# cambridge-mlg/RECOMBINER

Measured on AMD Instinct MI355X. Metric: INRs trained/sec (whole node) + PSNR@bpp vs reference, CIFAR-10, higher is better.
Workload: dtype bf16; 1 GPU; CIFAR-10 32x32, 4096 INRs/GPU, 3x32 SIREN (in 32 = 16 Fourier + 16 upsampled pe), S=1, training_mappings=True, Adam lr 2e-4; inrs_per_gpu=4096, parallelism=datapoint-sharded x1, tuned_library_gemms=True

## Files before the change

### recombiner_amd/csrc/atrans.hip

```cpp
#include "rcb_common.h"
#include "prepare_bodies.h"

#include <algorithm>
#include <type_traits>
#include <vector>

using namespace rcb;

namespace {

typedef __bf16 bf16x8 __attribute__((ext_vector_type(8)));
typedef float f32x16 __attribute__((ext_vector_type(16)));
typedef float f32x4 __attribute__((ext_vector_type(4)));

#ifndef ATRANS_DIAG
#define ATRANS_DIAG 0
#endif
#ifndef ATRANS_STAMPS
#define ATRANS_STAMPS 0
#endif
#ifndef ATRANS_SPREAD_PIN
#define ATRANS_SPREAD_PIN 1
#endif
constexpr int BM = 256, BK = 32, NT = 512, MAXL = RCB_ATRANS_MAX_LAYERS, MAXSEG = 7;
constexpr int XT_BYTES = BM * BK * 4;

__device__ __forceinline__ constexpr int rho(int r, int h) { return (r & 3) + 8 * (r >> 2) + 4 * h; }
__device__ __forceinline__ int xswz(int row, int c) { return row * 128 + ((c ^ ((row >> 1) & 7)) << 4); }
__device__ __forceinline__ int bswz(int row, int c) { return row * 64 + ((c ^ ((row >> 2) & 3)) << 4); }

typedef __attribute__((address_space(3))) void* lds_ptr_t;
__device__ __forceinline__ void dma16(const void* g, char* l) {
  __builtin_amdgcn_global_load_lds(g, (lds_ptr_t)l, 16, 0, 0);
}
__device__ __forceinline__ f32x16 mma(bf16x8 a, bf16x8 b, f32x16 c) {
#if ATRANS_DIAG == 4
  asm volatile("" ::"v"(a), "v"(b));
  return c;
#else
  return __builtin_amdgcn_mfma_f32_32x32x16_bf16(a, b, c, 0, 0, 0);
#endif
}
template <int N>
__device__ __forceinline__ void wait_vm() { asm volatile("s_waitcnt vmcnt(%0)" ::"n"(N) : "memory"); }
#if ATRANS_STAMPS
__device__ unsigned long long g_stamps[8][40][6];
#define STAMP(it, pt)                                                                 \
  do {                                                                               \
    if (blockIdx.x == 0 && (it) < 40) {                                              \
      const unsigned long long t_ = __builtin_amdgcn_s_memtime();                    \
      if (lane == 0) g_stamps[wave][it][pt] = t_;                                    \
    }                                                                                \
  } while (0)
#else
#define STAMP(it, pt)
#endif

struct AtArgs {
  const float* x;
  const __bf16* xh;
  const __bf16* xl;
  long long ld_x16;
  float* out;
  long long ld_x, ld_out, rows;
  int n_layers;
  int L[MAXL], Lp[MAXL], off[MAXL];
  const __bf16* bh[MAXL];
  const __bf16* bl[MAXL];
  const int4* segs;
  const int* seg_begin;
  int n_wg;
  int nt_out;
  float* ws;
  long long ld_ws;
};

template <int NCB, int TERMS>
struct Geo {
  static constexpr int NBW = (2 * NCB + 7) / 8;
  static constexpr int NDMA = 4 + NBW * (TERMS == 3 ? 2 : 1);
  static constexpr int BH_OFF = XT_BYTES;
  static constexpr int BT_BYTES = NCB * 32 * BK * 2;
  static constexpr int BL_OFF = BH_OFF + BT_BYTES;
  static constexpr int STAGE = BH_OFF + (TERMS == 3 ? 2 : 1) * BT_BYTES;
  static constexpr int NSTAGE = TERMS == 3 ? 2 : 3;
};
constexpr int LDS_MAX_BYTES = 3 * (XT_BYTES + MAXSEG * 32 * BK * 2);

template <int NCB, int TERMS, bool RAGGED, bool PLANES>
__device__ __forceinline__ void run_segment(const AtArgs& a, const int4 sg, const int4 sk, char* __restrict__ lds) {
  typedef Geo<NCB, TERMS> G;
  const int t = threadIdx.x, lane = t & 63;
  const int wave = __builtin_amdgcn_readfirstlane(t >> 6);
  const int l = sg.x, row0 = sg.y, cb0 = sg.z, ncb = sg.w;
  const int K = a.L[l], Lp = a.Lp[l];
  const int kc0 = sk.x, nk = sk.y - sk.x;
  const __bf16* __restrict__ bh = a.bh[l];
  const __bf16* __restrict__ bl = a.bl[l];
  const float* __restrict__ xl0 = PLANES ? nullptr : a.x + a.off[l];

  f32x16 acc[NCB];
#pragma unroll
  for (int i = 0; i < NCB; ++i)
#pragma unroll
    for (int q = 0; q < 16; ++q) acc[i][q] = 0.f;

  const float* xsrc[4];
  const __bf16* psrc[4];
  int xk[4];
#pragma unroll
  for (int i = 0; i < 4; ++i) {
    if (PLANES) {
      const int row = 32 * wave + 16 * (i & 1) + (lane >> 2);
      const int c = (lane & 3) ^ ((row >> 2) & 3);
      const long long gr = min((long long)row0 + row, a.rows - 1);
      psrc[i] = ((i >> 1) ? a.xl : a.xh) + gr * a.ld_x16 + a.off[l];
      xk[i] = 8 * c;
      xsrc[i] = nullptr;
    } else {
      const int row = 32 * wave + 8 * i + (lane >> 3);
      const int c = (lane & 7) ^ ((row >> 1) & 7);
      const long long gr = min((long long)row0 + row, a.rows - 1);
      xsrc[i] = xl0 + gr * a.ld_x;
      xk[i] = 4 * c;
      psrc[i] = nullptr;
    }
  }
  const __bf16* bsrc[G::NBW];
  const __bf16* bsrc2[G::NBW];
  int bdst[G::NBW];
#pragma unroll
  for (int j = 0; j < G::NBW; ++j) {
    const int d = min(wave + 8 * j, 2 * NCB - 1);
    const int row = 16 * d + (lane >> 2);
    const int c = (lane & 3) ^ ((row >> 2) & 3);
    const int grow = min(cb0 * 32 + row, Lp - 1);
    bsrc[j] = bh + (long long)grow * Lp + 8 * c;
    bsrc2[j] = bl + (long long)grow * Lp + 8 * c;
    bdst[j] = __builtin_amdgcn_readfirstlane(d * 1024);
  }
  auto issue_one = [&](int kc_, int i) {
    char* __restrict__ st = lds + (kc_ % G::NSTAGE) * G::STAGE;
    const int kc = ATRANS_DIAG == 2 ? 0 : kc0 + kc_;
    if (i < 4) {
      if (PLANES) {
        const int k = RAGGED ? 0 : min(kc * BK + xk[i], K - 8);
        dma16(psrc[i] + k, st + (i >> 1) * (XT_BYTES / 2) + (32 * wave + 16 * (i & 1)) * 64);
      } else {
        const int k = RAGGED ? 0 : min(kc * BK + xk[i], K - 4);
        dma16(xsrc[i] + k, st + (32 * wave + 8 * i) * 128);
      }
    } else if (TERMS == 3) {
      const int j = (i - 4) >> 1;
      if ((i - 4) & 1) dma16(bsrc2[j] + kc * BK, st + G::BL_OFF + bdst[j]);
      else dma16(bsrc[j] + kc * BK, st + G::BH_OFF + bdst[j]);
    } else {
      dma16(bsrc[i - 4] + kc * BK, st + G::BH_OFF + bdst[i - 4]);
    }
  };
  auto issue = [&](int kc) {
#pragma unroll
    for (int i = 0; i < G::NDMA; ++i) issue_one(kc, i);
  };

  const int frow = lane & 31, fh = lane >> 5;
  const int xrow = 32 * wave + frow;
  bf16x8 xh[2], xlo[2];
  f32x4 raw[4];
  auto x_read = [&](const char* __restrict__ st) {
    if (PLANES) {
#pragma unroll
      for (int q = 0; q < 4; ++q)
        if (TERMS >= 2 || q < 2)
          raw[q] = *reinterpret_cast<const f32x4*>(st + (q >> 1) * (XT_BYTES / 2) + bswz(xrow, 2 * (q & 1) + fh));
    } else {
#pragma unroll
      for (int q = 0; q < 4; ++q) raw[q] = *reinterpret_cast<const f32x4*>(st + xswz(xrow, 4 * (q >> 1) + 2 * fh + (q & 1)));
    }
  };
  auto x_convert = [&](int q) {
    if (PLANES) {
      if (q < 2) xh[q] = __builtin_bit_cast(bf16x8, raw[q]);
      else if (TERMS >= 2) xlo[q - 2] = __builtin_bit_cast(bf16x8, raw[q]);
      return;
    }
#pragma unroll
    for (int i = 0; i < 4; ++i) {
      const float v = raw[q][i];
      const __bf16 hb = (__bf16)v;
      xh[q >> 1][4 * (q & 1) + i] = hb;
      if (TERMS >= 2) xlo[q >> 1][4 * (q & 1) + i] = (__bf16)(v - (float)hb);
    }
  };
  constexpr int NBT = G::NDMA - 4;
  constexpr int CBR = (NCB - 1) / 2;
  auto compute = [&](const char* __restrict__ cur, const char* __restrict__ nxt, int kn, auto issue_c, auto pref_c) {
    constexpr bool ISSUE = decltype(issue_c)::value, PREF = decltype(pref_c)::value;
    bf16x8 b0 = *reinterpret_cast<const bf16x8*>(cur + G::BH_OFF + bswz(frow, fh));
    bf16x8 b1 = *reinterpret_cast<const bf16x8*>(cur + G::BH_OFF + bswz(frow, 2 + fh));
#pragma unroll
    for (int cb = 0; cb < NCB; ++cb) {
      const bf16x8 c0 = b0, c1 = b1;
      if (cb + 1 < NCB) {
        b0 = *reinterpret_cast<const bf16x8*>(cur + G::BH_OFF + bswz((cb + 1) * 32 + frow, fh));
        b1 = *reinterpret_cast<const bf16x8*>(cur + G::BH_OFF + bswz((cb + 1) * 32 + frow, 2 + fh));
      }
      acc[cb] = mma(xh[0], c0, acc[cb]);
      if (TERMS >= 2) acc[cb] = mma(xlo[0], c0, acc[cb]);
      acc[cb] = mma(xh[1], c1, acc[cb]);
      if (TERMS >= 2) acc[cb] = mma(xlo[1], c1, acc[cb]);
      if (TERMS == 3) {
        const int bo0 = bswz(cb * 32 + frow, fh), bo1 = bswz(cb * 32 + frow, 2 + fh);
        const bf16x8 d0 = *reinterpret_cast<const bf16x8*>(cur + G::BL_OFF + bo0);
        const bf16x8 d1 = *reinterpret_cast<const bf16x8*>(cur + G::BL_OFF + bo1);
        acc[cb] = mma(xh[0], d0, acc[cb]);
        acc[cb] = mma(xh[1], d1, acc[cb]);
      }
      if (ISSUE && ATRANS_DIAG != 6) {
#pragma unroll
        for (int i = cb * G::NDMA / NCB; i < (cb + 1) * G::NDMA / NCB; ++i) issue_one(kn, i);
      }
      if (PREF) {
        if (cb == CBR) {
          STAMP(kn - 2, 3);
          wait_vm<NBT + (ISSUE ? (CBR + 1) * G::NDMA / NCB : 0)>();
          x_read(nxt);
        }
      }
#if ATRANS_SPREAD_PIN
      __builtin_amdgcn_sched_barrier(0);
#endif
    }
    if (PREF) {
      STAMP(kn - 2, 4);
#pragma unroll
      for (int q = 0; q < 4; ++q) x_convert(q);
    }
  };
  auto yes = std::integral_constant<bool, true>{};
  auto no = std::integral_constant<bool, false>{};

  if (RAGGED) {
    for (int kr = 0; kr < nk; ++kr) {
      const int kc = kc0 + kr;
      __syncthreads();
#pragma unroll
      for (int j = 0; j < G::NBW; ++j) {
        dma16(bsrc[j] + kc * BK, lds + G::BH_OFF + bdst[j]);
        if (TERMS == 3) dma16(bsrc2[j] + kc * BK, lds + G::BL_OFF + bdst[j]);
      }
#pragma unroll
      for (int i = 0; i < 4; ++i) {
        const int k0 = kc * BK + xk[i];
        if (PLANES) {
          const int row = 32 * wave + 16 * (i & 1) + (lane >> 2), pc = lane & 3;
          const bool rok = (long long)row0 + row < a.rows;
          bf16x8 v;
#pragma unroll
          for (int e = 0; e < 8; ++e) v[e] = (rok && k0 + e < K) ? psrc[i][k0 + e] : (__bf16)0.f;
          *reinterpret_cast<bf16x8*>(lds + (i >> 1) * (XT_BYTES / 2) + row * 64 + pc * 16) = v;
        } else {
          const int row = 32 * wave + 8 * i + (lane >> 3), pc = lane & 7;
          const bool rok = (long long)row0 + row < a.rows;
          f32x4 v;
#pragma unroll
          for (int e = 0; e < 4; ++e) v[e] = (rok && k0 + e < K) ? xsrc[i][k0 + e] : 0.f;
          *reinterpret_cast<f32x4*>(lds + row * 128 + pc * 16) = v;
        }
      }
      wait_vm<0>();
      __syncthreads();
      x_read(lds);
#pragma unroll
      for (int q = 0; q < 4; ++q) x_convert(q);
      compute(lds, lds, -1, no, no);
    }
    __syncthreads();
  } else if (G::NSTAGE == 2) {
    issue(0);
    for (int kc = 0; kc < nk; ++kc) {
      wait_vm<0>();
      __builtin_amdgcn_s_barrier();
      __builtin_amdgcn_sched_barrier(0);
      const char* cur = lds + (kc & 1) * G::STAGE;
      x_read(cur);
#pragma unroll
      for (int q = 0; q < 4; ++q) x_convert(q);
      if (kc + 1 < nk) compute(cur, cur, kc + 1, yes, no);
      else compute(cur, cur, -1, no, no);
    }
    __builtin_amdgcn_s_barrier();
  } else {
    issue(0);
    if (nk > 1) {
      issue(1);
      wait_vm<G::NDMA + NBT>();
    } else {
      wait_vm<NBT>();
    }
    x_read(lds);
#pragma unroll
    for (int q = 0; q < 4; ++q) x_convert(q);
    int kc = 0;
    for (; kc + 2 < nk; ++kc) {
      STAMP(kc, 0);
      wait_vm<G::NDMA>();
      STAMP(kc, 1);
      __builtin_amdgcn_s_barrier();
      __builtin_amdgcn_sched_barrier(0);
      STAMP(kc, 2);
      if (ATRANS_DIAG != 3) compute(lds + (kc % 3) * G::STAGE, lds + ((kc + 1) % 3) * G::STAGE, kc + 2, yes, yes);
      else issue(kc + 2);
      STAMP(kc, 5);
    }
    if (kc + 1 < nk) {
      wait_vm<G::NDMA>();
      __builtin_amdgcn_s_barrier();
      __builtin_amdgcn_sched_barrier(0);
      if (ATRANS_DIAG != 3) compute(lds + (kc % 3) * G::STAGE, lds + ((kc + 1) % 3) * G::STAGE, -1, no, yes);
      ++kc;
    }
    wait_vm<0>();
    __builtin_amdgcn_s_barrier();
    __builtin_amdgcn_sched_barrier(0);
    if (ATRANS_DIAG != 3) compute(lds + (kc % 3) * G::STAGE, lds, -1, no, no);
    __builtin_amdgcn_s_barrier();
  }

  const bool direct = sk.z < 0;
  float* __restrict__ ob = (direct ? a.out : a.ws + (long long)sk.z * a.rows * a.ld_ws) + a.off[l];
  const long long ldo = direct ? a.ld_out : a.ld_ws;
#pragma unroll
  for (int cb = 0; cb < NCB; ++cb) {
    if (cb < ncb && (ATRANS_DIAG != 1 || a.rows < 0)) {
      const int col = (cb0 + cb) * 32 + frow;
      if (col < K) {
#pragma unroll
        for (int q = 0; q < 16; ++q) {
          const long long row = (long long)row0 + 32 * wave + rho(q, fh);
          if (row < a.rows) {
            if (a.nt_out) __builtin_nontemporal_store(acc[cb][q], ob + row * ldo + col);
            else ob[row * ldo + col] = acc[cb][q];
          }
        }
      }
    }
  }
}

template <int TERMS, bool RAGGED, bool PLANES>
__device__ __forceinline__ void dispatch_upto4(const AtArgs& a, const int4 sg, const int4 sk, char* lds) {
  switch (sg.w) {
    case 1: run_segment<1, TERMS, RAGGED, PLANES>(a, sg, sk, lds); break;
    case 2: run_segment<2, TERMS, RAGGED, PLANES>(a, sg, sk, lds); break;
    case 3: run_segment<3, TERMS, RAGGED, PLANES>(a, sg, sk, lds); break;
    default: run_segment<4, TERMS, RAGGED, PLANES>(a, sg, sk, lds); break;
  }
}

template <int TERMS, bool RAGGED, bool PLANES>
__device__ __forceinline__ void dispatch_segment(const AtArgs& a, const int4 sg, const int4 sk, char* lds) {
  if constexpr (TERMS == 3) {
    if (sg.w > 4) {
      const int n1 = (sg.w + 1) / 2;
      dispatch_upto4<TERMS, RAGGED, PLANES>(a, make_int4(sg.x, sg.y, sg.z, n1), sk, lds);
      dispatch_upto4<TERMS, RAGGED, PLANES>(a, make_int4(sg.x, sg.y, sg.z + n1, sg.w - n1), sk, lds);
    } else {
      dispatch_upto4<TERMS, RAGGED, PLANES>(a, sg, sk, lds);
    }
    return;
  }
  switch (sg.w) {
    case 1: run_segment<1, TERMS, RAGGED, PLANES>(a, sg, sk, lds); break;
    case 2: run_segment<2, TERMS, RAGGED, PLANES>(a, sg, sk, lds); break;
    case 3: run_segment<3, TERMS, RAGGED, PLANES>(a, sg, sk, lds); break;
    case 4: run_segment<4, TERMS, RAGGED, PLANES>(a, sg, sk, lds); break;
    case 5: run_segment<5, TERMS, RAGGED, PLANES>(a, sg, sk, lds); break;
    case 6: run_segment<6, TERMS, RAGGED, PLANES>(a, sg, sk, lds); break;
    default: run_segment<7, TERMS, RAGGED, PLANES>(a, sg, sk, lds); break;
  }
}

template <int TERMS, bool PLANES>
__global__ void __launch_bounds__(NT, 2) atrans_kernel(AtArgs a) {
  extern __shared__ __attribute__((aligned(16))) char lds[];
  int id = blockIdx.x;
  if ((a.n_wg & 7) == 0) id = (id & 7) * (a.n_wg >> 3) + (id >> 3);
  const int s0 = a.seg_begin[id], s1 = a.seg_begin[id + 1];
  for (int s = s0; s < s1; ++s) {
    const int4 sg = a.segs[2 * s], sk = a.segs[2 * s + 1];
    if (a.L[sg.x] & 7) {
      if (sg.w > 1) run_segment<2, TERMS, true, PLANES>(a, sg, sk, lds);
      else run_segment<1, TERMS, true, PLANES>(a, sg, sk, lds);
    } else {
      dispatch_segment<TERMS, false, PLANES>(a, sg, sk, lds);
    }
  }
}

struct SlabArgs {
  const float* ws;
  float* out;
  long long rows, ld_ws, ld_out;
  int n_layers;
  int off[MAXL + 1], slabs[MAXL];
};

__global__ void __launch_bounds__(256) atrans_slab_sum_kernel(SlabArgs a) {
  const long long total = a.rows * a.off[a.n_layers];
  for (long long e = (long long)blockIdx.x * 256 + threadIdx.x; e < total; e += (long long)gridDim.x * 256) {
    const long long r = e / a.off[a.n_layers];
    const int c = (int)(e - r * a.off[a.n_layers]);
    int l = 0;
    while (l + 1 < a.n_layers && c >= a.off[l + 1]) ++l;
    float v = 0.f;
    for (int k = 0; k < a.slabs[l]; ++k) v += a.ws[((long long)k * a.rows + r) * a.ld_ws + c];
    a.out[r * a.ld_out + c] = v;
  }
}

__global__ void __launch_bounds__(256) atrans_pack_kernel(PackArgs a) { atrans_pack_body(a, (int)blockIdx.x); }


struct Blk {
  int layer, cb, w, maxseg;
};

long long run_cost(const std::vector<Blk>& blks, int b0, int b1, std::vector<int4>* segs, int row0) {
  long long cost = 0;
  int i = b0;
  while (i < b1) {
    int j = i;
    while (j < b1 && blks[j].layer == blks[i].layer) ++j;
    const int n = j - i, ms = blks[i].maxseg, parts = (n + ms - 1) / ms;
    int done = 0;
    for (int p = 0; p < parts; ++p) {
      const int m = (n - done + (parts - p) - 1) / (parts - p);
      cost += (long long)m * blks[i].w + 6;
      if (segs) segs->push_back(make_int4(blks[i].layer, row0, blks[i + done].cb, m));
      done += m;
    }
    i = j;
  }
  return cost;
}

}

extern "C" int64_t rcb_atrans_pack_elems(int32_t n_layers, const int32_t* sizes) {
  if (!sizes || n_layers < 1 || n_layers > MAXL) return -1;
  int64_t plane = 0;
  for (int l = 0; l < n_layers; ++l) plane += (int64_t)pad32(sizes[l]) * pad32(sizes[l]);
  return 4 * plane;
}

extern "C" int rcb_atrans_pack(const float* const* A, int32_t n_layers, const int32_t* sizes, void* packed, int32_t want_lo,
                               rcb_stream_t stream) {
  RCB_REQUIRE(A && sizes && packed && n_layers >= 1 && n_layers <= MAXL, RCB_ERR_ARG, "atrans_pack: bad arguments (%d layers)", n_layers);
  RCB_REQUIRE((reinterpret_cast<uintptr_t>(packed) & 15) == 0, RCB_ERR_ARG, "atrans_pack: packed buffer must be 16-byte aligned");
  for (int l = 0; l < n_layers; ++l) RCB_REQUIRE(A[l] && sizes[l] >= 1, RCB_ERR_ARG, "atrans_pack: layer %d null / empty", l);
  PackArgs a;
  const int tiles = fill_pack_args(a, A, n_layers, sizes, packed, want_lo);
  atrans_pack_kernel<<<tiles, 256, 0, (hipStream_t)stream>>>(a);
  RCB_LAUNCH_CHECK();
  return RCB_OK;
}

extern "C" int rcb_atrans_plan(int64_t rows, int32_t n_layers, const int32_t* sizes, int32_t n_cu, int32_t* plan,
                               int32_t max_ints) {
  RCB_REQUIRE(sizes && (plan || max_ints == 0) && n_layers >= 1 && n_layers <= MAXL && rows >= 1 && n_cu >= 1 && max_ints >= 0,
              RCB_ERR_ARG, "atrans_plan: bad arguments");
  std::vector<Blk> blks;
  for (int l = 0; l < n_layers; ++l) {
    RCB_REQUIRE(sizes[l] >= 1, RCB_ERR_ARG, "atrans_plan: layer %d empty", l);
    const int lp = pad32(sizes[l]);
    for (int cb = 0; cb < lp / 32; ++cb) blks.push_back(Blk{l, cb, lp / BK, (sizes[l] & 7) ? 2 : MAXSEG});
  }
  const int nb = (int)blks.size();
  const long long m_tiles = (rows + BM - 1) / BM;
  int R = (int)std::max<long long>(1, n_cu / m_tiles);
  R = std::min(R, (nb + 1) / 2);
  const int runs_full = (nb + MAXSEG - 1) / MAXSEG;
  int S = 1;
  if (m_tiles * runs_full * 2 <= n_cu) {
    S = (int)std::min<long long>(8, n_cu / (m_tiles * runs_full));
    R = runs_full;
  }
  long long lo = 0, hi = run_cost(blks, 0, nb, nullptr, 0);
  auto fits = [&](long long bound, std::vector<int>* cuts) {
    int b = 0, runs = 0;
    while (b < nb) {
      int e = b + 1;
      if (run_cost(blks, b, e, nullptr, 0) > bound) return false;
      while (e < nb && run_cost(blks, b, e + 1, nullptr, 0) <= bound) ++e;
      if (cuts) cuts->push_back(e);
      b = e;
      if (++runs > R) return false;
    }
    return true;
  };
  while (lo < hi) {
    const long long mid = (lo + hi) / 2;
    if (fits(mid, nullptr)) hi = mid; else lo = mid + 1;
  }
  std::vector<int> cuts;
  fits(hi, &cuts);
  const int runs = (int)cuts.size();
  std::vector<int4> segs;
  std::vector<int> begin;
  int slabs[MAXL];
  for (int l = 0; l < n_layers; ++l) slabs[l] = std::min(S, pad32(sizes[l]) / BK);
  for (long long mt = 0; mt < m_tiles; ++mt) {
    int b = 0;
    for (int ri = 0; ri < runs; ++ri) {
      std::vector<int4> run;
      run_cost(blks, b, cuts[ri], &run, (int)(mt * BM));
      b = cuts[ri];
      if (S == 1) {
        begin.push_back((int)segs.size() / 2);
        for (const int4& sg : run) {
          segs.push_back(sg);
          segs.push_back(make_int4(0, pad32(sizes[sg.x]) / BK, -1, 0));
        }
      } else {
        for (const int4& sg : run) {
          const int nc = pad32(sizes[sg.x]) / BK, sl = slabs[sg.x];
          for (int k = 0; k < sl; ++k) {
            begin.push_back((int)segs.size() / 2);
            segs.push_back(sg);
            segs.push_back(make_int4((int)((long long)k * nc / sl), (int)((long long)(k + 1) * nc / sl), k, 0));
          }
        }
      }
    }
  }
  begin.push_back((int)segs.size() / 2);
  const long long n_wg = (long long)begin.size() - 1;
  RCB_REQUIRE(n_wg < (1 << 24), RCB_ERR_SHAPE, "atrans_plan: %lld workgroups", n_wg);
  const long long head = ((RCB_ATRANS_PLAN_HEAD + n_wg + 1) + 3) / 4 * 4;
  const long long need = head + 4 * (long long)segs.size();
  RCB_REQUIRE(need < (1ll << 31), RCB_ERR_SHAPE, "atrans_plan: plan of %lld ints", need);
  if (max_ints == 0) return (int)need;
  if (need > max_ints) return rcb::fail(RCB_ERR_SHAPE, "atrans_plan: %lld ints needed, %d given", need, max_ints);
  memset(plan, 0, sizeof(int32_t) * head);
  plan[0] = (int32_t)n_wg;
  plan[1] = (int32_t)(segs.size() / 2);
  plan[2] = S;
  for (int l = 0; l < n_layers; ++l) plan[4 + l] = S == 1 ? 0 : slabs[l];
  for (size_t i = 0; i < begin.size(); ++i) plan[RCB_ATRANS_PLAN_HEAD + i] = begin[i];
  memcpy(plan + head, segs.data(), sizeof(int4) * segs.size());
  return (int)need;
}

extern "C" int rcb_atrans_apply(const float* x, int64_t ld_x, const void* x_hi, const void* x_lo, int64_t ld_x16, float* out,
                                int64_t ld_out, int64_t rows, int32_t n_layers, const int32_t* sizes, const void* packed,
                                int32_t transpose, int32_t terms, const int32_t* plan_dev, const int32_t* plan_head,
                                float* workspace, rcb_stream_t stream) {
  RCB_REQUIRE((x || x_hi) && out && sizes && packed && plan_dev && plan_head && n_layers >= 1 && n_layers <= MAXL && rows >= 1,
              RCB_ERR_ARG, "atrans_apply: bad arguments");
  const bool planes = x_hi != nullptr;
  RCB_REQUIRE(!planes || (x == nullptr && (x_lo != nullptr || terms == 1) && (ld_x16 & 7) == 0 &&
                          ((reinterpret_cast<uintptr_t>(x_hi) | reinterpret_cast<uintptr_t>(x_lo)) & 15) == 0),
              RCB_ERR_ARG, "atrans_apply: operand planes: give x_hi and x_lo (terms >= 2) INSTEAD of x, 16-byte aligned, row stride a multiple of 8");
  const int n_wg = plan_head[0], ksplit = plan_head[2];
  RCB_REQUIRE(n_wg >= 1 && ksplit >= 1 && ksplit <= 8 && (ksplit == 1 || workspace), RCB_ERR_ARG,
              "atrans_apply: plan head (workgroups %d, slices %d) / workspace", n_wg, ksplit);
  RCB_REQUIRE(terms >= 1 && terms <= 3, RCB_ERR_ARG, "atrans_apply: terms = %d (1..3)", terms);
  RCB_REQUIRE((reinterpret_cast<uintptr_t>(packed) & 15) == 0 && (reinterpret_cast<uintptr_t>(plan_dev) & 15) == 0, RCB_ERR_ARG,
              "atrans_apply: packed images / plan must be 16-byte aligned");
  AtArgs a;
  memset(&a, 0, sizeof(a));
  long long plane = 0, off = 0;
  for (int l = 0; l < n_layers; ++l) plane += (long long)pad32(sizes[l]) * pad32(sizes[l]);
  const __bf16* pk = reinterpret_cast<const __bf16*>(packed);
  long long poff = 0;
  for (int l = 0; l < n_layers; ++l) {
    a.L[l] = sizes[l];
    a.Lp[l] = pad32(sizes[l]);
    a.off[l] = (int)off;
    a.bh[l] = pk + (transpose ? plane : 0) + poff;
    a.bl[l] = pk + (transpose ? 3 : 2) * plane + poff;
    off += sizes[l];
    poff += (long long)a.Lp[l] * a.Lp[l];
  }
  RCB_REQUIRE((planes ? ld_x16 : ld_x) >= off && ld_out >= off, RCB_ERR_SHAPE, "atrans_apply: row strides %lld / %lld below %lld columns",
              (long long)(planes ? ld_x16 : ld_x), (long long)ld_out, off);
  if (planes)
    for (int l = 0; l < n_layers; ++l)
      RCB_REQUIRE((sizes[l] & 7) != 0 || (a.off[l] & 7) == 0, RCB_ERR_SHAPE, "atrans_apply: operand planes: layer %d starts at column %d (not a multiple of 8)", l, a.off[l]);
  a.x = x; a.out = out; a.ld_x = ld_x; a.ld_out = ld_out; a.rows = rows; a.n_layers = n_layers;
  a.xh = reinterpret_cast<const __bf16*>(x_hi);
  a.xl = reinterpret_cast<const __bf16*>(x_lo ? x_lo : x_hi);
  a.ld_x16 = ld_x16;
  a.nt_out = transpose ? 1 : 0;
  const long long head = ((RCB_ATRANS_PLAN_HEAD + (long long)n_wg + 1) + 3) / 4 * 4;
  a.seg_begin = plan_dev + RCB_ATRANS_PLAN_HEAD;
  a.segs = reinterpret_cast<const int4*>(plan_dev + head);
  a.n_wg = n_wg;
  a.ws = workspace;
  a.ld_ws = (off + 3) / 4 * 4;
  const int lds = LDS_MAX_BYTES;
  hipError_t e;
  auto go = [&](auto kfn) {
    e = hipFuncSetAttribute(reinterpret_cast<const void*>(kfn), hipFuncAttributeMaxDynamicSharedMemorySize, lds);
    if (e == hipSuccess) kfn<<<n_wg, NT, lds, (hipStream_t)stream>>>(a);
  };
  if (terms == 1) {
    if (planes) go(atrans_kernel<1, true>); else go(atrans_kernel<1, false>);
  } else if (terms == 2) {
    if (planes) go(atrans_kernel<2, true>); else go(atrans_kernel<2, false>);
  } else {
    if (planes) go(atrans_kernel<3, true>); else go(atrans_kernel<3, false>);
  }
  RCB_REQUIRE(e == hipSuccess, (int)e, "atrans_apply: hipFuncSetAttribute: %s", hipGetErrorString(e));
  RCB_LAUNCH_CHECK();
  if (ksplit > 1) {
    SlabArgs r;
    memset(&r, 0, sizeof(r));
    r.ws = workspace; r.out = out; r.rows = rows; r.ld_ws = a.ld_ws; r.ld_out = ld_out; r.n_layers = n_layers;
    for (int l = 0; l < n_layers; ++l) {
      r.off[l] = a.off[l];
      r.slabs[l] = plan_head[4 + l];
      RCB_REQUIRE(r.slabs[l] >= 1 && r.slabs[l] <= ksplit, RCB_ERR_ARG, "atrans_apply: plan head: %d slices for layer %d", r.slabs[l], l);
    }
    r.off[n_layers] = (int)off;
    long long blocks = (rows * off + 255) / 256;
    if (blocks > 4096) blocks = 4096;
    atrans_slab_sum_kernel<<<(int)blocks, 256, 0, (hipStream_t)stream>>>(r);
    RCB_LAUNCH_CHECK();
  }
  return RCB_OK;
}

extern "C" int64_t rcb_atrans_workspace_floats(int64_t rows, int32_t n_layers, const int32_t* sizes, const int32_t* plan_head) {
  if (!sizes || !plan_head || n_layers < 1 || n_layers > MAXL || rows < 1) return -1;
  if (plan_head[2] <= 1) return 0;
  long long off = 0;
  for (int l = 0; l < n_layers; ++l) off += sizes[l];
  return (int64_t)plan_head[2] * rows * ((off + 3) / 4 * 4);
}

namespace {
struct NarrowOp {
  const float* f;
  const __bf16* hi;
  const __bf16* lo;
  long long ld;
  __device__ __forceinline__ float at(long long m, int c) const {
    if (f) return f[m * ld + c];
    return (float)hi[m * ld + c] + (float)lo[m * ld + c];
  }
};

__global__ void __launch_bounds__(256) wgrad_narrow_kernel(NarrowOp hop, NarrowOp dop, long long rows, int L, int n_slabs,
                                                           float* __restrict__ part) {
  __shared__ float red[4][16][64];
  const int nt = (L + 31) / 32;
  const int tile = blockIdx.x % (nt * nt), slab = blockIdx.x / (nt * nt);
  const int k0 = (tile / nt) * 32, n0 = (tile % nt) * 32;
  const long long per = ((rows + n_slabs - 1) / n_slabs + 7) / 8 * 8;
  const long long m_begin = slab * per, m_end = min(rows, m_begin + per);
  const int t = threadIdx.x, wave = t >> 6, lane = t & 63, i = lane & 31, kh = lane >> 5;
  const bool kin = k0 + i < L, nin = n0 + i < L;
  const int hc = k0 + (kin ? i : 0), dc = n0 + (nin ? i : 0);
  f32x16 acc;
#pragma unroll
  for (int q = 0; q < 16; ++q) acc[q] = 0.f;
  for (long long m0 = m_begin + 2 * wave; m0 < m_end; m0 += 64) {
    float av[8], bv[8];
#pragma unroll
    for (int u = 0; u < 8; ++u) {
      const long long m = m0 + 8 * u + kh;
      const bool ok = m < m_end;
      const long long mc = ok ? m : m_begin;
      av[u] = hop.at(mc, hc);
      bv[u] = dop.at(mc, dc);
      av[u] = (ok && kin) ? av[u] : 0.f;
      bv[u] = (ok && nin) ? bv[u] : 0.f;
    }
#pragma unroll
    for (int u = 0; u < 8; ++u) acc = __builtin_amdgcn_mfma_f32_32x32x2f32(av[u], bv[u], acc, 0, 0, 0);
  }
#pragma unroll
  for (int q = 0; q < 16; ++q) red[wave][q][lane] = acc[q];
  __syncthreads();
  float* o = part + ((long long)slab * nt * nt + tile) * 1024;
#pragma unroll
  for (int j = 0; j < 4; ++j) {
    const int e = t + 256 * j, q = e >> 6, ln = e & 63;
    const float v = ((red[0][q][ln] + red[1][q][ln]) + red[2][q][ln]) + red[3][q][ln];
    o[rho(q, ln >> 5) * 32 + (ln & 31)] = v;
  }
}

__global__ void __launch_bounds__(256) wgrad_narrow_sum_kernel(const float* __restrict__ part, int L, int n_slabs, float* __restrict__ dA) {
  const int nt = (L + 31) / 32;
  const int i = blockIdx.x * 256 + threadIdx.x;
  if (i >= L * L) return;
  const int k = i / L, n = i - k * L;
  const int tile = (k >> 5) * nt + (n >> 5);
  const float* p = part + (long long)tile * 1024 + (k & 31) * 32 + (n & 31);
  float s = 0.f;
  const long long st = (long long)nt * nt * 1024;
  int sl = 0;
  for (; sl + 8 <= n_slabs; sl += 8) {
    float v[8];
#pragma unroll
    for (int u = 0; u < 8; ++u) v[u] = p[(sl + u) * st];
#pragma unroll
    for (int u = 0; u < 8; ++u) s += v[u];
  }
  for (; sl < n_slabs; ++sl) s += p[sl * st];
  dA[i] = s;
}
}

extern "C" int64_t rcb_atrans_wgrad_narrow_workspace(int32_t L, int32_t n_slabs) {
  if (L < 1 || n_slabs < 1) return -1;
  const int64_t nt = (L + 31) / 32;
  return (int64_t)n_slabs * nt * nt * 1024;
}

extern "C" int rcb_atrans_wgrad_narrow(const float* h, const void* h_hi, const void* h_lo, int64_t ld_h, const float* d,
                                       const void* d_hi, const void* d_lo, int64_t ld_d, int64_t rows, int32_t L, float* dA,
                                       float* workspace, int32_t n_slabs, rcb_stream_t stream) {
  RCB_REQUIRE(dA && workspace && rows >= 1 && L >= 1 && L <= 1024 && n_slabs >= 1 && n_slabs <= 4096, RCB_ERR_ARG,
              "atrans_wgrad_narrow: bad arguments (L = %d, slabs = %d)", L, n_slabs);
  RCB_REQUIRE((h != nullptr) != (h_hi != nullptr && h_lo != nullptr) && (d != nullptr) != (d_hi != nullptr && d_lo != nullptr), RCB_ERR_ARG,
              "atrans_wgrad_narrow: each operand either as fp32 rows or as a (hi, lo) pair of bf16 planes");
  RCB_REQUIRE(ld_h >= L && ld_d >= L, RCB_ERR_SHAPE, "atrans_wgrad_narrow: row strides below the layer size");
  const int nt = (L + 31) / 32;
  const NarrowOp hop{h, reinterpret_cast<const __bf16*>(h_hi), reinterpret_cast<const __bf16*>(h_lo), ld_h};
  const NarrowOp dop{d, reinterpret_cast<const __bf16*>(d_hi), reinterpret_cast<const __bf16*>(d_lo), ld_d};
  wgrad_narrow_kernel<<<nt * nt * n_slabs, 256, 0, (hipStream_t)stream>>>(hop, dop, rows, L, n_slabs, workspace);
  RCB_LAUNCH_CHECK();
  wgrad_narrow_sum_kernel<<<(L * L + 255) / 256, 256, 0, (hipStream_t)stream>>>(workspace, L, n_slabs, dA);
  RCB_LAUNCH_CHECK();
  return RCB_OK;
}

#if ATRANS_STAMPS
extern "C" int rcb_debug_atrans_stamps(unsigned long long* host, int32_t n) {
  if (n > 8 * 40 * 6) n = 8 * 40 * 6;
  hipError_t e = hipMemcpyFromSymbol(host, HIP_SYMBOL(g_stamps), sizeof(unsigned long long) * n);
  return (int)e;
}
#endif
```

Measured before the change: 72.94 INRs trained/s.

## Replace greedy atrans run partitioning with DP planner using fixed-cost model

Replaces the binary-search greedy split of column blocks into per-workgroup runs with a dynamic-programming planner. The planner uses a cost model that charges fixed per-segment overhead (higher for ragged layers) and, when K-splitting, caps the number of workgroups at the greedy count. The aim is better load balance and less per-segment overhead across CUs in the atrans kernel. It also adds optional per-workgroup timestamp instrumentation behind ATRANS_STAMPS, and the new cost constants are heuristic.

```diff
diff --git a/recombiner_amd/csrc/atrans.hip b/recombiner_amd/csrc/atrans.hip
--- a/recombiner_amd/csrc/atrans.hip
+++ b/recombiner_amd/csrc/atrans.hip
@@ -45,6 +45,8 @@
 __device__ __forceinline__ void wait_vm() { asm volatile("s_waitcnt vmcnt(%0)" ::"n"(N) : "memory"); }
 #if ATRANS_STAMPS
 __device__ unsigned long long g_stamps[8][40][6];
+constexpr int WG_STAMPS = 8192;
+__device__ unsigned long long g_wg_stamps[WG_STAMPS][4];
 #define STAMP(it, pt)                                                                 \
   do {                                                                               \
     if (blockIdx.x == 0 && (it) < 40) {                                              \
@@ -386,6 +388,9 @@
   extern __shared__ __attribute__((aligned(16))) char lds[];
   int id = blockIdx.x;
   if ((a.n_wg & 7) == 0) id = (id & 7) * (a.n_wg >> 3) + (id >> 3);
+#if ATRANS_STAMPS
+  const unsigned long long rt0 = __builtin_amdgcn_s_memrealtime(), ct0 = __builtin_amdgcn_s_memtime();
+#endif
   const int s0 = a.seg_begin[id], s1 = a.seg_begin[id + 1];
   for (int s = s0; s < s1; ++s) {
     const int4 sg = a.segs[2 * s], sk = a.segs[2 * s + 1];
@@ -396,6 +401,16 @@
       dispatch_segment<TERMS, false, PLANES>(a, sg, sk, lds);
     }
   }
+#if ATRANS_STAMPS
+  wait_vm<0>();
+  __syncthreads();
+  if (threadIdx.x == 0 && id < WG_STAMPS) {
+    g_wg_stamps[id][0] = rt0;
+    g_wg_stamps[id][1] = __builtin_amdgcn_s_memrealtime();
+    g_wg_stamps[id][2] = ct0;
+    g_wg_stamps[id][3] = __builtin_amdgcn_s_memtime();
+  }
+#endif
 }
 
 struct SlabArgs {
@@ -422,12 +437,41 @@
 __global__ void __launch_bounds__(256) atrans_pack_kernel(PackArgs a) { atrans_pack_body(a, (int)blockIdx.x); }
 
 
+constexpr int PLAN_F = 3, PLAN_E = 28, PLAN_F_RAGGED = 20;
+
 struct Blk {
-  int layer, cb, w, maxseg;
+  int layer, cb, w, maxseg, wgs, nc, f;
 };
 
-long long run_cost(const std::vector<Blk>& blks, int b0, int b1, std::vector<int4>* segs, int row0) {
-  long long cost = 0;
+struct Piece {
+  long long cost;
+  int segs, wgs;
+};
+Piece piece_cost(const Blk& b, int n, bool ksplit) {
+  const int parts = (n + b.maxseg - 1) / b.maxseg;
+  if (ksplit) return Piece{(long long)b.w * (b.f + (n + parts - 1) / parts) + PLAN_E, parts, parts * b.wgs};
+  return Piece{(long long)b.w * ((long long)b.f * parts + n) + (long long)PLAN_E * parts, parts, 1};
+}
+
+template <class Fn>
+void runs_ending_at(const std::vector<Blk>& blks, int e, bool ksplit, Fn fn) {
+  long long tail = 0;
+  int tail_segs = 0, tail_wgs = 0, n = 0;
+  for (int b = e - 1; b >= 0; --b) {
+    if (n && blks[b].layer != blks[b + 1].layer) {
+      const Piece p = piece_cost(blks[b + 1], n, ksplit);
+      tail = ksplit ? std::max(tail, p.cost) : tail + p.cost;
+      tail_segs += p.segs;
+      tail_wgs += p.wgs;
+      n = 0;
+    }
+    ++n;
+    const Piece p = piece_cost(blks[b], n, ksplit);
+    if (!fn(b, ksplit ? std::max(tail, p.cost) : tail + p.cost, tail_segs + p.segs, ksplit ? tail_wgs + p.wgs : 1)) break;
+  }
+}
+
+void run_segments(const std::vector<Blk>& blks, int b0, int b1, std::vector<int4>& segs, int row0) {
   int i = b0;
   while (i < b1) {
     int j = i;
@@ -436,13 +480,119 @@
     int done = 0;
     for (int p = 0; p < parts; ++p) {
       const int m = (n - done + (parts - p) - 1) / (parts - p);
-      cost += (long long)m * blks[i].w + 6;
-      if (segs) segs->push_back(make_int4(blks[i].layer, row0, blks[i + done].cb, m));
+      segs.push_back(make_int4(blks[i].layer, row0, blks[i + done].cb, m));
       done += m;
     }
     i = j;
   }
-  return cost;
+}
+
+long long greedy_workgroups(const std::vector<Blk>& blks, int R) {
+  const int nb = (int)blks.size();
+  auto run = [&](int b0, int b1, long long* wgs) {
+    long long cost = 0;
+    for (int i = b0, j; i < b1; i = j) {
+      for (j = i; j < b1 && blks[j].layer == blks[i].layer;) ++j;
+      const int parts = (j - i + blks[i].maxseg - 1) / blks[i].maxseg;
+      cost += (long long)(j - i) * blks[i].nc + 6 * parts;
+      if (wgs) *wgs += (long long)parts * blks[i].wgs;
+    }
+    return cost;
+  };
+  auto fits = [&](long long bound, long long* wgs) {
+    int b = 0, runs = 0;
+    while (b < nb) {
+      int e = b + 1;
+      if (run(b, e, nullptr) > bound) return false;
+      while (e < nb && run(b, e + 1, nullptr) <= bound) ++e;
+      run(b, e, wgs);
+      b = e;
+      if (++runs > R) return false;
+    }
+    return true;
+  };
+  long long lo = 0, hi = run(0, nb, nullptr);
+  while (lo < hi) {
+    const long long mid = (lo + hi) / 2;
+    if (fits(mid, nullptr)) hi = mid; else lo = mid + 1;
+  }
+  long long wgs = 0;
+  fits(hi, &wgs);
+  return wgs;
+}
+
+std::vector<int> plan_cuts(const std::vector<Blk>& blks, int R, bool ksplit, long long wg_budget) {
+  const int nb = (int)blks.size();
+  const int INF = 1 << 30;
+  struct Best {
+    int extra;
+    long long sq;
+    int from;
+  };
+  const Best none{INF, 0, -1};
+  std::vector<std::vector<Best>> best;
+  auto solve = [&](long long bound) {
+    best.assign(R + 1, std::vector<Best>(nb + 1, none));
+    best[0][0] = Best{0, 0, 0};
+    for (int r = 1; r <= R; ++r)
+      for (int e = r; e <= nb; ++e)
+        runs_ending_at(blks, e, ksplit, [&](int b, long long cost, int segs, int wgs) {
+          if (cost <= bound && best[r - 1][b].extra < INF) {
+            const Best c{best[r - 1][b].extra + (ksplit ? wgs : segs - 1), best[r - 1][b].sq + cost * cost, b};
+            Best& t = best[r][e];
+            if (c.extra < t.extra || (c.extra == t.extra && c.sq < t.sq)) t = c;
+          }
+          return ksplit || cost <= bound;
+        });
+    int fewest = INF;
+    for (int r = 1; r <= R; ++r) fewest = std::min(fewest, best[r][nb].extra);
+    return fewest < INF && (!ksplit || fewest <= wg_budget);
+  };
+  if (ksplit) {
+    std::vector<long long> cand;
+    for (int i = 0; i < nb; ++i)
+      if (i == 0 || blks[i].layer != blks[i - 1].layer)
+        for (int m = 1; m <= blks[i].maxseg; ++m) cand.push_back(piece_cost(blks[i], m, true).cost);
+    std::sort(cand.begin(), cand.end());
+    size_t lo = 0, hi = cand.size() - 1;
+    while (lo < hi) {
+      const size_t mid = (lo + hi) / 2;
+      if (solve(cand[mid])) hi = mid; else lo = mid + 1;
+    }
+    solve(cand[hi]);
+  } else {
+    auto fits = [&](long long bound) {
+      int e = nb, runs = 0;
+      while (e > 0) {
+        int first = e;
+        runs_ending_at(blks, e, false, [&](int b, long long cost, int, int) {
+          if (cost <= bound) first = b;
+          return cost <= bound;
+        });
+        if (first == e || ++runs > R) return false;
+        e = first;
+      }
+      return true;
+    };
+    long long lo = 0, hi = 0;
+    runs_ending_at(blks, nb, false, [&](int, long long cost, int, int) { hi = cost; return true; });
+    while (lo < hi) {
+      const long long mid = (lo + hi) / 2;
+      if (fits(mid)) hi = mid; else lo = mid + 1;
+    }
+    solve(hi);
+  }
+  int runs = 0;
+  for (int r = 1; r <= R; ++r) {
+    const Best &c = best[r][nb], &t = best[runs][nb];
+    if (c.extra < INF && (runs == 0 || c.extra < t.extra || (c.extra == t.extra && c.sq <= t.sq))) runs = r;
+  }
+  std::vector<int> cuts(runs);
+  for (int r = runs, e = nb; r >= 1; --r) {
+    cuts[r - 1] = e;
+    e = best[r][e].from;
+  }
+  return cuts;
 }
 
 }
@@ -470,13 +620,11 @@
                                int32_t max_ints) {
   RCB_REQUIRE(sizes && (plan || max_ints == 0) && n_layers >= 1 && n_layers <= MAXL && rows >= 1 && n_cu >= 1 && max_ints >= 0,
               RCB_ERR_ARG, "atrans_plan: bad arguments");
-  std::vector<Blk> blks;
+  int nb = 0;
   for (int l = 0; l < n_layers; ++l) {
     RCB_REQUIRE(sizes[l] >= 1, RCB_ERR_ARG, "atrans_plan: layer %d empty", l);
-    const int lp = pad32(sizes[l]);
-    for (int cb = 0; cb < lp / 32; ++cb) blks.push_back(Blk{l, cb, lp / BK, (sizes[l] & 7) ? 2 : MAXSEG});
-  }
-  const int nb = (int)blks.size();
+    nb += pad32(sizes[l]) / 32;
+  }
   const long long m_tiles = (rows + BM - 1) / BM;
   int R = (int)std::max<long long>(1, n_cu / m_tiles);
   R = std::min(R, (nb + 1) / 2);
@@ -486,35 +634,24 @@
     S = (int)std::min<long long>(8, n_cu / (m_tiles * runs_full));
     R = runs_full;
   }
-  long long lo = 0, hi = run_cost(blks, 0, nb, nullptr, 0);
-  auto fits = [&](long long bound, std::vector<int>* cuts) {
-    int b = 0, runs = 0;
-    while (b < nb) {
-      int e = b + 1;
-      if (run_cost(blks, b, e, nullptr, 0) > bound) return false;
-      while (e < nb && run_cost(blks, b, e + 1, nullptr, 0) <= bound) ++e;
-      if (cuts) cuts->push_back(e);
-      b = e;
-      if (++runs > R) return false;
-    }
-    return true;
-  };
-  while (lo < hi) {
-    const long long mid = (lo + hi) / 2;
-    if (fits(mid, nullptr)) hi = mid; else lo = mid + 1;
-  }
-  std::vector<int> cuts;
-  fits(hi, &cuts);
+  int slabs[MAXL];
+  for (int l = 0; l < n_layers; ++l) slabs[l] = std::min(S, pad32(sizes[l]) / BK);
+  std::vector<Blk> blks;
+  for (int l = 0; l < n_layers; ++l) {
+    const int lp = pad32(sizes[l]), nc = lp / BK;
+    const bool ragged = (sizes[l] & 7) != 0;
+    for (int cb = 0; cb < lp / 32; ++cb)
+      blks.push_back(Blk{l, cb, (nc + slabs[l] - 1) / slabs[l], ragged ? 2 : MAXSEG, slabs[l], nc, ragged ? PLAN_F_RAGGED : PLAN_F});
+  }
+  const std::vector<int> cuts = plan_cuts(blks, R, S > 1, S > 1 ? greedy_workgroups(blks, R) : 0);
   const int runs = (int)cuts.size();
   std::vector<int4> segs;
   std::vector<int> begin;
-  int slabs[MAXL];
-  for (int l = 0; l < n_layers; ++l) slabs[l] = std::min(S, pad32(sizes[l]) / BK);
   for (long long mt = 0; mt < m_tiles; ++mt) {
     int b = 0;
     for (int ri = 0; ri < runs; ++ri) {
       std::vector<int4> run;
-      run_cost(blks, b, cuts[ri], &run, (int)(mt * BM));
+      run_segments(blks, b, cuts[ri], run, (int)(mt * BM));
       b = cuts[ri];
       if (S == 1) {
         begin.push_back((int)segs.size() / 2);
@@ -745,4 +882,10 @@
   hipError_t e = hipMemcpyFromSymbol(host, HIP_SYMBOL(g_stamps), sizeof(unsigned long long) * n);
   return (int)e;
 }
+
+extern "C" int rcb_debug_atrans_wg_stamps(unsigned long long* host, int32_t n_wg) {
+  if (n_wg > WG_STAMPS) n_wg = WG_STAMPS;
+  hipError_t e = hipMemcpyFromSymbol(host, HIP_SYMBOL(g_wg_stamps), sizeof(unsigned long long) * 4 * n_wg);
+  return (int)e;
+}
 #endif
```

After: 75.00 INRs trained/s, median of 6. 2.8% higher.
